# fan-ziqi/robot_lab

Measured on AMD Instinct MI355X. Metric: env-steps/sec (whole node) at 4096 envs/GPU, A1 Velocity-Rough, higher is better.
Workload: dtype f32; 1 GPU; RobotLab-Isaac-Velocity-Rough-Unitree-A1-v0, 4096 envs/GPU, random actions U(-1,1), seed 42+rank; envs_per_gpu=4096, parallelism=env-shard x1, step_kernel=specialised (spec_id 1), envs_per_wavefront=4

## Files before the change

__graft_entry__.py:

```python
from __future__ import annotations

import os
import subprocess
import sys

ROOT = os.path.dirname(os.path.abspath(__file__))
CSRC = os.path.join(ROOT, "robot_lab_amd", "csrc")
HIP_LIB = os.path.join(CSRC, "librl_env_hip.so")
EMU_DIR = os.path.join(ROOT, "tests", "emu")
EMU_LIB = os.path.join(EMU_DIR, "librl_env_emu.so")
HEADERS = ["rl_math.h", "env_tables.h", "env_step.h", "env_terms.h", "env_aos.h", "rl_env_host.h", "rl_env_capi.inl", "rl_env_kernels.h", "rl_env_sub.inl",
           "env_spec.h", "rl_env_spec.inl", "rl_env_specgen.h", os.path.join("spec", "env_specs_gen.h")]
ENV_SOURCES = ["rl_env.hip", "rl_env_sub1.hip", "rl_env_sub2.hip", "rl_env_sub8.hip"] + sorted(
    os.path.join("spec", f) for f in os.listdir(os.path.join(CSRC, "spec")) if f.startswith("rl_env_spec_") and f.endswith(".hip"))


def _stale(target, sources):
    if not os.path.isfile(target):
        return True
    t = os.path.getmtime(target)
    return any(os.path.getmtime(s) > t for s in sources)


_ONLY_MISSING = False
# ... 3 lines not shown
    return not os.path.isfile(target) if _ONLY_MISSING else _stale(target, sources)


VALIDATED_HIPCC = "HIP version: 7.2.26015-fc0010cf6a"
BUILD_INFO = os.path.join(CSRC, "build_info.json")


def _record_compiler(hipcc: str, extra: dict | None = None) -> None:
    import json

    try:
        ver = subprocess.run([hipcc, "--version"], capture_output=True, text=True, check=True).stdout.strip().splitlines()
    except (OSError, subprocess.CalledProcessError):
        ver = ["unknown"]
    ok = bool(ver) and ver[0].strip() == VALIDATED_HIPCC
    with open(BUILD_INFO, "w") as f:
        json.dump({"hipcc": hipcc, "version": ver[:2], "validated": VALIDATED_HIPCC, "matches_validated": ok,
                   "flags": " ".join(ENV_FLAGS), **(extra or {})}, f, indent=1)
    if not ok:
        print(f"[build] WARNING: hipcc reports {ver[0]!r}, the env library was validated with {VALIDATED_HIPCC!r}: run the GPU parity "
              f"tier and tests/test_gpu_canary.py before trusting this build", flush=True)


ENV_FLAGS = ["--offload-arch=gfx950", "-O3", "-fno-slp-vectorize", "-fno-signed-zeros", "-ffinite-math-only", "-mllvm", "-amdgpu-remove-redundant-endcf=false", "-std=c++17"]


def _abi_stamp_flag() -> str:
    if ROOT not in sys.path:
        sys.path.insert(0, ROOT)
    from robot_lab_amd import jit

    return jit.stamp_flag()


def _build_env_library(hipcc: str) -> None:
    import importlib.util
    import shutil
    import tempfile

    spec = importlib.util.spec_from_file_location("isa_exec_hazard", os.path.join(ROOT, "tools", "isa_exec_hazard.py"))
    chk = importlib.util.module_from_spec(spec)
    spec.loader.exec_module(chk)
    with tempfile.TemporaryDirectory(prefix="rl_env_build_") as tmp:
        procs = []
        for src in ENV_SOURCES:
            d = os.path.join(tmp, os.path.basename(src)[:-4])
            os.makedirs(d)
# ... 265 lines not shown
```

robot_lab_amd/csrc/env_step.h:

```cpp
#pragma once
#include <type_traits>

#include "env_spec.h"
#include "env_tables.h"

#if !defined(RL_NO_PK) && !defined(RL_PK)
#define RL_PK 1
#endif
#if defined(RL_PHASE_MARKS) && defined(__HIP_DEVICE_COMPILE__)
#define RL_PHASE(id, name) asm volatile("; PHASE " name)
#elif defined(RL_PHASE_CLOCK) && defined(__HIP_DEVICE_COMPILE__)
#define RL_PHASE(id, name) this->phase_stamp(id)
#define RL_PHASE_START() (this->ph_t0 = 0, this->ph_cur = 0)
#define RL_PHASE_CLOCK_ON 1
#else
#define RL_PHASE(id, name) ((void)0)
#endif
#ifndef RL_PHASE_START
#define RL_PHASE_START() ((void)0)
#endif
constexpr int RL_PHASE_ROW0 = 24;
constexpr int RL_PHASE_SLOTS = 32;

namespace rl {
// ... 83 lines not shown
struct TerrainPatch {
  float h00, h01, h10, h11, fx, fy;
};
struct TerrainBase {
  int cx, cy;
  float fx, fy;
  float lox, hix, loy, hiy;
};
RL_FN TerrainBase terrain_base(const Uni& u, float bx, float by) {
  TerrainBase b;
  if (u.is_plane) {
    b.cx = b.cy = 0;
    b.fx = b.fy = b.lox = b.hix = b.loy = b.hiy = 0.f;
    return b;
  }
  const double gx = ((double)bx - u.x0d) * u.inv_hd, gy = ((double)by - u.y0d) * u.inv_hd;
  const double cx = floor(gx), cy = floor(gy);
  b.cx = (int)cx; b.cy = (int)cy;
  b.fx = (float)(gx - cx); b.fy = (float)(gy - cy);
  b.lox = (float)(-b.cx); b.hix = (float)(u.nx - 2 - b.cx);
  b.loy = (float)(-b.cy); b.hiy = (float)(u.ny - 2 - b.cy);
  return b;
}
RL_FN TerrainPatch terrain_fetch(const Uni& u, const float* __restrict__ hf, const TerrainBase& tb, float dx, float dy) {
  TerrainPatch p;
  if (u.is_plane) {
    p.h00 = p.h01 = p.h10 = p.h11 = 0.f;
    p.fx = p.fy = 0.f;
    return p;
  }
  const float gx = tb.fx + dx * u.inv_hscale, gy = tb.fy + dy * u.inv_hscale;
  const float ox = clampf(floorf(gx), tb.lox, tb.hix), oy = clampf(floorf(gy), tb.loy, tb.hiy);
  p.fx = clampf(gx - ox, 0.f, 1.f);
  p.fy = clampf(gy - oy, 0.f, 1.f);
  const int ix = imin(imax(tb.cx + (int)ox, 0), u.nx - 2), iy = imin(imax(tb.cy + (int)oy, 0), u.ny - 2);
  if constexpr (TERRAIN_PAIRS) {
    const F4h r = ld4_a8(hf + (((uint32_t)ix * (uint32_t)u.ny + (uint32_t)iy) << 1));
    p.h00 = r.x; p.h10 = r.y; p.h01 = r.z; p.h11 = r.w;
  } else {
    const float* b = hf + (uint32_t)ix * (uint32_t)u.ny + (uint32_t)iy;
    F2 r0 = ld2(b), r1 = ld2(b + u.ny);
    p.h00 = r0.x; p.h01 = r0.y; p.h10 = r1.x; p.h11 = r1.y;
  }
  return p;
}
RL_FN TerrainPatch terrain_fetch(const Uni& u, const float* __restrict__ hf, float bx, float by, float dx, float dy) {
  return terrain_fetch(u, hf, terrain_base(u, bx, by), dx, dy);
}
RL_FN void terrain_eval(const Uni& u, const TerrainPatch& p, float& h, V3& n) {
  float hx0 = p.h00 + p.fx * (p.h10 - p.h00), hx1 = p.h01 + p.fx * (p.h11 - p.h01);
  h = hx0 + p.fy * (hx1 - hx0);
  float dzdx = ((1.f - p.fy) * (p.h10 - p.h00) + p.fy * (p.h11 - p.h01)) * u.inv_hscale;
  float dzdy = ((1.f - p.fx) * (p.h01 - p.h00) + p.fx * (p.h11 - p.h10)) * u.inv_hscale;
  float inv = frsqrt(dzdx * dzdx + dzdy * dzdy + 1.0f);
  n = {-dzdx * inv, -dzdy * inv, inv};
}
RL_FN float terrain_height(const TerrainPatch& p) {
  const float hx0 = p.h00 + p.fx * (p.h10 - p.h00), hx1 = p.h01 + p.fx * (p.h11 - p.h01);
// ... 2141 lines not shown
```

robot_lab_amd/csrc/env_terms.h:

```cpp
#pragma once
#include "env_spec.h"
#include "env_step.h"

namespace rl {

enum RewKind {
  REW_TRACK_LIN_VEL_XY_EXP = 0, REW_TRACK_ANG_VEL_Z_EXP, REW_LIN_VEL_Z_L2, REW_ANG_VEL_XY_L2, REW_JOINT_TORQUES_L2,
  REW_JOINT_ACC_L2, REW_JOINT_POS_LIMITS, REW_JOINT_POWER, REW_STAND_STILL, REW_JOINT_POS_PENALTY, REW_JOINT_MIRROR,
  REW_ACTION_RATE_L2, REW_UNDESIRED_CONTACTS, REW_CONTACT_FORCES, REW_FEET_CONTACT_WITHOUT_CMD, REW_FEET_HEIGHT_BODY,
  REW_UPWARD, REW_FEET_AIR_TIME, REW_FEET_AIR_TIME_VARIANCE, REW_FEET_SLIDE, REW_FEET_GAIT, REW_FLAT_ORIENTATION_L2,
  REW_IS_TERMINATED, REW_JOINT_DEVIATION_L1, REW_JOINT_VEL_L2, REW_FEET_CONTACT, REW_FEET_STUMBLE, REW_FEET_HEIGHT,
  REW_TRACK_LIN_VEL_XY_YAW_FRAME_EXP, REW_TRACK_ANG_VEL_Z_WORLD_EXP, REW_FEET_AIR_TIME_POSITIVE_BIPED,
  REW_HANDSTAND_FEET_HEIGHT_EXP, REW_HANDSTAND_FEET_ON_AIR, REW_HANDSTAND_FEET_AIR_TIME, REW_HANDSTAND_ORIENTATION_L2, REW_BASE_HEIGHT_L2, REW_WHEEL_VEL_PENALTY,
  REW_FEET_DISTANCE_Y_EXP, REW_FEET_DISTANCE_XY_EXP, REW_ACTION_MIRROR, REW_ACTION_SYNC
};
enum ObsKind {
  OBS_BASE_LIN_VEL = 0, OBS_BASE_ANG_VEL, OBS_PROJECTED_GRAVITY, OBS_VELOCITY_COMMANDS, OBS_JOINT_POS_REL,
  OBS_JOINT_VEL_REL, OBS_LAST_ACTION, OBS_HEIGHT_SCAN, OBS_JOINT_POS_REL_NO_WHEEL
};

enum { JS_TAU2 = 0, JS_ACC2, JS_QD2, JS_LIMIT, JS_POWER, JS_DEV1, JS_DEV2, JS_DA2, JS_Q, JS_ABSQD, JS_ROWS };
enum { BT_HMAX = 0, BT_CA, BT_CC, BT_LA, BT_LC, BT_FX, BT_FY, BT_FZ, BT_PX, BT_PY, BT_PZ, BT_VX, BT_VY, BT_VZ, BT_NF };
static_assert(JS_ROWS == REW_JS_ROWS && BT_NF == REW_BT_NF && BT_FX == REW_BT_NS, "reward tables: LDS sizing in env_tables.h");

// ... 276 lines not shown
        case REW_UNDESIRED_CONTACTS: f = a0 * gate; break;
        case REW_CONTACT_FORCES: f = a0; break;
        case REW_FEET_CONTACT_WITHOUT_CMD: f = a0 * (cmd_norm < 0.1f ? 1.f : 0.f) * gate; break;
        case REW_FEET_CONTACT: f = (a0 != R.p[0] ? 1.f : 0.f) * moving * gate; break;
        case REW_FEET_AIR_TIME: f = a0 * moving * gate; break;
        case REW_HANDSTAND_FEET_AIR_TIME: f = a0; break;
        case REW_FEET_STUMBLE: f = (a0 > 0.f ? 1.f : 0.f) * gate; break;
        case REW_FEET_HEIGHT_BODY: case REW_FEET_HEIGHT: f = a0 * moving * gate; break;
        case REW_FEET_SLIDE: f = a0 * gate; break;
        case REW_FEET_AIR_TIME_POSITIVE_BIPED: f = (a0 == 1.f ? fminf(mn, R.p[0]) : 0.f) * moving * gate; break;
        case REW_HANDSTAND_FEET_HEIGHT_EXP: f = fexp(-a0 * frcp(R.p[0])); break;
        case REW_HANDSTAND_FEET_ON_AIR: f = a0 == 0.f ? 1.f : 0.f; break;
        case REW_FEET_AIR_TIME_VARIANCE: {
          const float inv_n = frcp(a0), inv_den = frcp(fmaxf(a0 - 1.f, 1.f));
          f = ((a2 - a1 * a1 * inv_n) + (a4 - a3 * a3 * inv_n)) * inv_den * gate;
        } break;
        default: break;
      }
    } break;
  }
  return f;
}


template <class Ctx, class TP, class SP = NoSpec>
struct EnvProgram : EnvLane<Ctx, TP, SP> {
  using Base = EnvLane<Ctx, TP, SP>;
  using ChainTP = typename Base::ChainTP;
  static constexpr Layout LY = Base::LY;
  static constexpr int CL = TP::CL, NW = TP::NW, JX = TP::JX, NBS = TP::NBS;
  using Base::ctx; using Base::S; using Base::T; using Base::L; using Base::e; using Base::k; using Base::sub; using Base::li; using Base::Np;
  static constexpr int SUB = Base::SUB;
  static constexpr int LPE = Base::LPE;
  using Base::pos; using Base::quat; using Base::vlin; using Base::vang; using Base::q; using Base::qd; using Base::kp; using Base::kd;
  using Base::act; using Base::prev_act; using Base::tim; using Base::cf; using Base::hist_n; using Base::tau_app; using Base::qacc;
  using Base::extF; using Base::extT; using Base::base_com; using Base::wr_com;

  V3 cmd;
  float heading_target, cmd_time_left, metric_xy, metric_yaw, push_left;
  static constexpr bool DEFER_LOG = SUB > 1;
  static constexpr int NACC_M = (MAX_T + LPE - 1) / LPE;
  float log_sum[NACC_M], log_mxy, log_myaw;
  bool is_heading, is_standing;
  int level, ttype;
  V3 origin;
  long long ep_len;
// ... 682 lines not shown

  RL_FN void scanner_pose(float& cy, float& sy, V3& scan_p, bool chain_fresh) {
    if (NW == 0) {
      cy = yaw_c; sy = yaw_s; scan_p = {0.f, 0.f, pos.z};
      return;
    }
    M3 Rf;
    V3 pf;
    if (chain_fresh) {
      ChainTP C = this->new_chain();
      trunk_frame<TP>(C, T.scan_depth, Rf, pf);
    } else {
      RL_PHASE(31, "obs.kinematics");
      trunk_frame_of_pose<TP>(L, q, this->u.trunk_restart, T.scan_depth, Rf, pf);
      RL_PHASE(20, "observations");
    }
    const M3 Rs = mul(Rwb, Rf);
    const float hn = frsqrt(fmaxf(Rs.r0.x * Rs.r0.x + Rs.r1.x * Rs.r1.x, 1e-30f));
    cy = Rs.r0.x * hn; sy = Rs.r1.x * hn;
    const V3 so = mul(Rwb, pf + mul(Rf, V3{T.scan_pos[0], T.scan_pos[1], T.scan_pos[2]}));
    scan_p = {so.x, so.y, pos.z + so.z};
  }

  static constexpr int SCAN_RB = LPE >= 32 ? 6 : 12;
  struct ScanPatches {
    TerrainPatch tp[SCAN_RB];
    bool single_trip;
  };
  RL_FN int scan_ray_of_slot(int s, int scan_n, float cy, float sy) const {
    s = s < scan_n ? s : scan_n - 1;
#ifndef RL_SCAN_YAW_LANES
    return s;
#else
    const int snx = ctx.uniform_i(T.scan_nx);
    const float inv_sny = ctx.uniform(1.0f / (float)T.scan_ny);
    const int ixt = (int)(((float)s + 0.5f) * inv_sny), iyt = s - ixt * ctx.uniform_i(T.scan_ny);
    return fabsf(cy) > fabsf(sy) ? iyt * snx + ixt : s;
#endif
  }
  RL_FN void scan_fetch_trip(int r0, int scan_n, float cy, float sy, V3 scan_p, ScanPatches& sp) const {
    const TerrainBase tb = terrain_base(this->u, pos.x, pos.y);
    const int snx = ctx.uniform_i(T.scan_nx);
    const float inv_snx = ctx.uniform(1.0f / (float)T.scan_nx);
    const float res = T.scan_res, cx0 = 0.5f * (float)(T.scan_nx - 1), cy0 = 0.5f * (float)(T.scan_ny - 1);
#pragma unroll
    for (int i = 0; i < SCAN_RB; ++i) {
      const int r = scan_ray_of_slot(r0 + i * LPE, scan_n, cy, sy);
      int iy = (int)(((float)r + 0.5f) * inv_snx), ix = r - iy * snx;
      float lx = ((float)ix - cx0) * res, ly = ((float)iy - cy0) * res;
      sp.tp[i] = terrain_fetch(this->u, S.terrain, tb, scan_p.x + cy * lx - sy * ly, scan_p.y + sy * lx + cy * ly);
    }
  }
  RL_FN void scan_fetch(float cy, float sy, V3 scan_p, ScanPatches& sp) const {
    const int scan_n = ctx.uniform_i(T.scan_nx * T.scan_ny);
    const bool wanted = ctx.uniform_i(T.obs[0].scan_n + T.obs[1].scan_n) > 0;
    sp.single_trip = wanted && scan_n <= SCAN_RB * LPE;
#ifdef RL_ABL_NO_SCAN
    sp.single_trip = false;
#endif
    if (sp.single_trip) scan_fetch_trip(li, scan_n, cy, sy, scan_p, sp);
  }

  template <bool DIRECT, class GT>
  RL_FN void write_group(const GT& G, const float* F, float* stage, uint32_t noise_base, float cy, float sy, V3 scan_p, const ScanPatches& sp) {
    constexpr int NITC = (TP::OBS_NC + LPE - 1) / LPE;
#ifdef RL_ABL_NO_SCAN
    const int n_cols = ctx.uniform_i(G.n_cols), scan_off = ctx.uniform_i(G.scan_off), scan_n = 0;
#else
    const int n_cols = ctx.uniform_i(G.n_cols), scan_off = ctx.uniform_i(G.scan_off), scan_n = ctx.uniform_i(G.scan_n);
#endif
    const int dim = ctx.uniform_i(G.dim);
    const bool corrupt = !DIRECT && ctx.uniform_i(G.corrupt) != 0;
    {
      ObsColTab d[NITC];
      float f[NITC];
#pragma unroll
      for (int i = 0; i < NITC; ++i) {
        const int n = li + LPE * i;
        d[i] = G.col[n < n_cols ? n : 0];
      }
#pragma unroll
      for (int i = 0; i < NITC; ++i) f[i] = F[d[i].src];
#pragma unroll
      for (int i = 0; i < NITC; ++i) {
        const int n = li + LPE * i;
        if (n < n_cols) stage[n < scan_off ? n : n + scan_n] = corrupt ? f[i] : clampf(f[i], d[i].clip_lo, d[i].clip_hi) * d[i].scale;
      }
    }
    if (scan_n > 0) write_scan(stage, scan_off, scan_n, corrupt, ctx.uniform(G.scan.scale), ctx.uniform(G.scan.clip_lo), ctx.uniform(G.scan.clip_hi), cy, sy, scan_p, sp);
    if (corrupt) noise_pass(G, stage, noise_base, dim, scan_off, scan_n);
  }
  RL_FN void write_scan(float* stage, int scan_off, int scan_n, bool corrupt, float s_scale, float s_lo, float s_hi, float cy, float sy, V3 scan_p,
                        const ScanPatches& sp) {
    const float soff = T.scan_offset;
    if (sp.single_trip) {
#pragma unroll
      for (int i = 0; i < SCAN_RB; ++i) {
        const int sl = li + i * LPE, r = scan_ray_of_slot(sl, scan_n, cy, sy);
        const float v = scan_p.z - terrain_height(sp.tp[i]) - soff;
        if (sl < scan_n) stage[scan_off + r] = corrupt ? v : clampf(v, s_lo, s_hi) * s_scale;
      }
    } else {
      for (int r0 = li; r0 < scan_n; r0 += SCAN_RB * LPE) {
        ScanPatches one;
        scan_fetch_trip(r0, scan_n, cy, sy, scan_p, one);
#pragma unroll
        for (int i = 0; i < SCAN_RB; ++i) {
          const int sl = r0 + i * LPE, r = scan_ray_of_slot(sl, scan_n, cy, sy);
          const float v = scan_p.z - terrain_height(one.tp[i]) - soff;
          if (sl < scan_n) stage[scan_off + r] = corrupt ? v : clampf(v, s_lo, s_hi) * s_scale;
        }
      }
    }
  }
  template <class GT>
  RL_FN void noise_pass(const GT& G, float* stage, uint32_t noise_base, int dim, int scan_off, int scan_n) {
    ctx.group_sync();
    const int nblk = (dim + 3) >> 2;
#pragma unroll 1
    for (int b = li; b < nblk; b += LPE) {
      float un[4];
      uniform01x4(S.seed, (uint32_t)e, S.step_counter, STREAM_NOISE, (noise_base >> 2) + (uint32_t)b, un);
// ... 146 lines not shown
      int b = L.slot_body[s];
      if (b >= 0 && (s != 0 || L.owns_base_body) && this->owns_slot(s)) {
        float* o = S.dbg_cforce + ((size_t)e * T.n_bodies + b) * 3;
        const F4 fs = cf.ld(s);
        o[0] = live * fs.x; o[1] = live * fs.y; o[2] = live * fs.z;
      }
    }
  }
  RL_FN bool out_of_bounds() const {
    if (!T.term_oob || T.is_plane) return false;
    const float mw = (float)T.num_rows * T.tile_size + 2.f * T.border, mh = (float)T.num_cols * T.tile_size + 2.f * T.border;
    return fabsf(pos.x) > 0.5f * mw - T.oob_buffer || fabsf(pos.y) > 0.5f * mh - T.oob_buffer;
  }

  RL_FN void step() { step_front<false>(); }
  RL_FN void step_head() { step_front<true>(); }
  RL_FN void step_tail() {
    this->load();
    load_task();
    derive();
    const bool terminated = S.terminated[e] != 0, time_out = S.time_out[e] != 0;
    const bool t_oob = out_of_bounds();
    const bool t_timeout = T.term_time_out && ep_len >= (long long)T.max_episode_length;
    step_back<true>(terminated, time_out, t_timeout, t_oob, terminated);
  }

  template <bool HEAD>
  RL_FN void step_front() {
    constexpr size_t LOG_SLOT_WORDS = (size_t)LOG_PARTS * LOG_SIZE;
    const int log_tl = ctx.tile(), log_wl = ctx.env_in_tile() * LPE + li;
    float* log_pv = S.log + (size_t)((S.step_counter - 1u) & (uint32_t)(LOG_RING - 1)) * LOG_SLOT_WORDS;
    const float* log_pp = S.log + (size_t)((S.step_counter - 2u) & (uint32_t)(LOG_RING - 1)) * LOG_SLOT_WORDS;
    float log_fresh = 0.f, log_word = 0.f;
    if (log_tl < LOG_PARTS) {
      for (int p = 0; p < LOG_PARTS; ++p) log_fresh += log_pv[p * LOG_SIZE + LOG_FRESH];
      log_word = log_pp[log_tl * LOG_SIZE + log_wl];
    }
    float a_in[JX];
    {
      const float* arow = S.action_in + (size_t)(e < S.N ? e : 0) * T.D;
#pragma unroll
      for (int j = 0; j < JX; ++j) {
        const int jid = L.joint_id[j];
        a_in[j] = arow[TP::PAD && jid < 0 ? 0 : jid];
      }
    }
    RL_PHASE_START();
// ... 16 lines not shown
#pragma unroll
    for (int j = 0; j < JX; ++j) {
      prev_act[j] = act[j];
      const float a = (e < S.N && (!TP::PAD || L.joint_id[j] >= 0)) ? a_in[j] : 0.f;
      act[j] = a;
      float pr = clampf(a * L.a_scale[j] + L.a_off[j], L.a_lo[j], L.a_hi[j]);
      q_tgt[j] = L.action_is_vel[j] ? 0.f : pr;
      qd_tgt[j] = L.action_is_vel[j] ? pr : 0.f;
    }
#ifdef RL_ABL_SUBSTEPS
    if constexpr (Base::ABA) {
      this->substeps_aba(q_tgt, qd_tgt, RL_ABL_SUBSTEPS);
    } else
#endif
    if constexpr (Base::ABA) {
      this->substeps_aba(q_tgt, qd_tgt, T.decimation);
    } else {
      this->self_load();
      for (int s = 0; s < T.decimation; ++s) this->substep_aba_trunk(q_tgt, qd_tgt);
    }
    RL_PHASE(15, "terminations");
    ep_len += 1;
    derive();
    if constexpr (NW > 0) {
      ChainTP Cf = this->new_chain();
      this->kinematics(Cf);
      ctx.group_sync();
    }

    bool t_timeout = T.term_time_out && ep_len >= (long long)T.max_episode_length;
    const bool t_oob = out_of_bounds();
    bool t_illegal = false;
    if (T.term_illegal) {
      const uint64_t ill_mask = T.illegal_body_mask;
      const float ill_thr = T.illegal_threshold;
      float c = 0.f;
#pragma unroll
      for (int i = 0; i < Base::MAXOWN; ++i) {
        const int so = this->own[i], s = so < 0 ? 0 : so;
        const float h = hist_max(s);
        const bool bit = body_bit(ill_mask, s);
        c += (so >= 0 && bit && h > ill_thr) ? 1.f : 0.f;
      }
      t_illegal = ctx.esum(c) > 0.f;
    }
    bool terminated = t_illegal, time_out = t_timeout || t_oob;
// ... 8 lines not shown
    else rew = compute_rewards(terminated, fold_done);
#endif
    RL_PHASE(19, "resets+commands+push");
    if (li == 0) {
      S.reward[e] = rew;
      S.terminated[e] = terminated ? 1 : 0;
      S.time_out[e] = time_out ? 1 : 0;
      if (S.ro_rewards != nullptr && e < S.N) {
        if (S.ro_values != nullptr) {
          S.ro_rewards[e] = time_out ? fmaf(S.ro_gamma, S.ro_values[e], rew) : rew;
          S.ro_dones[e] = (terminated || time_out) ? 1 : 0;
        } else {
          S.ro_rewards[e] = rew;
          S.ro_dones[e] = ((terminated || time_out) ? 1 : 0) | (time_out ? 2 : 0);
        }
      }
    }
    if constexpr (HEAD) {
      collect_cmd_levels(terminated || time_out);
      write_dbg_views((terminated || time_out) ? 0.f : 1.f);
      this->store();
      store_task();
    } else {
      step_back<false>(terminated, time_out, t_timeout, t_oob, t_illegal, fold_done);
    }
  }

  template <bool TAIL>
  RL_FN void step_back(const bool terminated, const bool time_out, const bool t_timeout, const bool t_oob, const bool t_illegal, const bool sums_folded = false) {
    if (terminated || time_out) {
      if (!(DEFER_LOG && sums_folded) && li == 0 && e < S.N) {
        if (t_timeout) ctx.atomic_add(log_slot() + LOG_TERM_TIMEOUT, 1.f);
        if (t_oob) ctx.atomic_add(log_slot() + LOG_TERM_OOB, 1.f);
        if (t_illegal) ctx.atomic_add(log_slot() + LOG_TERM_ILLEGAL, 1.f);
      }
      reset_env(true, sums_folded);
      derive();
      RL_PHASE(19, "resets+commands+push");
    }
    if constexpr (!TAIL) write_dbg_views((terminated || time_out) ? 0.f : 1.f);
#ifdef RL_SCAN_EARLY
    ScanAhead scanA;
    scan_ahead(!TAIL && !ctx.any(terminated || time_out), scanA);
#endif
    RL_PHASE(29, "commands");
    {
      const float inv_max_step = T.step_dt * frcp(T.cmd_resample[1]);
      float ex = cmd.x - lin_b.x, ey = cmd.y - lin_b.y;
      metric_xy += fsqrt(ex * ex + ey * ey) * inv_max_step;
      metric_yaw += fabsf(cmd.z - ang_b.z) * inv_max_step;
      cmd_time_left -= T.step_dt;
      if (cmd_time_left <= 0.f) {
        cmd_time_left = U(STREAM_COMMAND, 6, T.cmd_resample[0], T.cmd_resample[1]);
        resample_command(STREAM_COMMAND, 0);
      }
      if (T.cmd_heading && is_heading) {
        const float heading_w = atan2f(yaw_s, yaw_c);
        cmd.z = clampf(T.cmd_heading_stiffness * wrap_to_pi(heading_target - heading_w), T.cur_ang ? S.cmd_levels[CL_ANG_Z] : T.cmd_range[2][0],
                       T.cur_ang ? S.cmd_levels[CL_ANG_Z + 1] : T.cmd_range[2][1]);
      }
      if (is_standing) cmd = {0.f, 0.f, 0.f};
    }
    RL_PHASE(30, "push");
    if (T.ev_push) {
      push_left -= T.step_dt;
      if (push_left < 1e-6f) {
        push_left = U(STREAM_PUSH, 6, T.push_interval[0], T.push_interval[1]);
        vlin += V3{U(STREAM_PUSH, 0, T.push_vel[0][0], T.push_vel[0][1]), U(STREAM_PUSH, 1, T.push_vel[1][0], T.push_vel[1][1]),
                   U(STREAM_PUSH, 2, T.push_vel[2][0], T.push_vel[2][1])};
        vang += V3{U(STREAM_PUSH, 3, T.push_vel[3][0], T.push_vel[3][1]), U(STREAM_PUSH, 4, T.push_vel[4][0], T.push_vel[4][1]),
                   U(STREAM_PUSH, 5, T.push_vel[5][0], T.push_vel[5][1])};
      }
    }
    RL_PHASE(23, "store");
#ifndef RL_ABL_NO_STORE
    this->store();
    store_task();
#endif
    RL_PHASE(20, "observations");
#ifndef RL_ABL_NO_OBS
#ifdef RL_SCAN_EARLY
    observations(scanA);
#else
    observations(!TAIL && !ctx.any(terminated || time_out));
#endif
#endif
#ifndef RL_ABL_NO_LOG
    if constexpr (DEFER_LOG) {
      if (sums_folded && e < S.N) {
        float* slot = log_slot();
        int n_rew;
        if constexpr (SP::ON) n_rew = SP::N_REW;
        else n_rew = T.n_rewards;
#pragma unroll
        for (int i = 0; i < NACC_M; ++i) {
          const int t = li + LPE * i;
          if (t < n_rew) ctx.atomic_add(slot + LOG_EP_SUM0 + t, log_sum[i]);
        }
        if (li == 0) {
          ctx.atomic_add(slot + LOG_RESET_COUNT, 1.0f);
          ctx.atomic_add(slot + LOG_FRESH, 1.0f);
          ctx.atomic_add(slot + LOG_METRIC_XY, log_mxy);
          ctx.atomic_add(slot + LOG_METRIC_YAW, log_myaw);
          if (t_timeout) ctx.atomic_add(slot + LOG_TERM_TIMEOUT, 1.f);
          if (t_oob) ctx.atomic_add(slot + LOG_TERM_OOB, 1.f);
          if (t_illegal) ctx.atomic_add(slot + LOG_TERM_ILLEGAL, 1.f);
        }
      }
// ... 23 lines not shown
```

robot_lab_amd/csrc/rl_env.hip:

```cpp
#include <dlfcn.h>

#include <mutex>

#include "rl_env_kernels.h"
#include "rl_env_host.h"
#include "rl_env_specgen.h"

#define RL_ENV_PLUGINS 1
#ifndef RL_ENV_ABI_STAMP
#define RL_ENV_ABI_STAMP "unstamped"
#endif
namespace {
struct SpecPlugin {
  int id = 0;
  int (*matches)(const void* tables) = nullptr;
  int (*launch)(const void* cfg, const void* S, const void* T, int sub, size_t lds1, void* stream) = nullptr;
};
std::vector<SpecPlugin>& spec_plugins() {
  static std::vector<SpecPlugin> v;
  return v;
}
std::mutex& spec_plugins_mutex() {
  static std::mutex m;
  return m;
// ... 125 lines not shown
        case 4: need[0] = lds_need<TopoQuad4, 4>(T); need[1] = lds_need<TopoQuad4, 2>(T); need[2] = lds_need<TopoQuad4, 1>(T); break;
        case 104: need[0] = lds_need<TopoQuad4M, 4>(T); need[1] = lds_need<TopoQuad4M, 2>(T); need[2] = lds_need<TopoQuad4M, 1>(T); break;
        default: break;
      }
      const int subs[3] = {4, 2, 1};
      const double cost[3] = {1.0, 1.45, 2.29};
      double best = 0.0, t[3] = {0.0, 0.0, 0.0};
      for (int i = 0; i < 3; ++i) {
        if (need[i] == 0 || need[i] > 160 * 1024) continue;
        const size_t per_cu = (tb + 4 * (need[i] - tb) <= 160 * 1024) ? 4 : std::min<size_t>(4, (160 * 1024) / need[i]);
        const double slots = (double)n_cu * (double)per_cu, waves = (double)(Npad / (16 / subs[i]));
        t[i] = cost[i] * std::ceil(waves / slots);
        if (best == 0.0 || t[i] < 0.97 * best) { best = t[i]; sub = subs[i]; }
      }
      if (std::getenv("RL_ENV_DEBUG"))
        fprintf(stderr, "rl_env: %d envs: rounds x cost of 4 / 2 / 1 lanes per limb = %.2f / %.2f / %.2f (LDS per wavefront %zu / %zu / %zu B, tables %zu B) -> %d lane(s) per limb\n",
                Npad, t[0], t[1], t[2], need[0], need[1], need[2], tb, sub);
    }
    return 16 / sub;
  }
  size_t lds_bytes = 0;
  template <class TP, int SUB>
  static size_t lds_need(const Tables& T) {
    const LdsPlan P = lds_plan<TP, SUB>(T.policy_dim, T.critic_dim, direct_group(T, 0), direct_group(T, 1), T.D, T.n_bodies, T.rew_ext_mask, T.n_rewards);
    return staged_bytes(T) + (size_t)P.words * 4;
  }
  int configure(const Tables& T) {
    const int key = (T.CL + (T.merged ? 100 : 0) + (T.NW > 3 ? 200 : 0) + (T.rotpad ? 400 : 0)) * 10 + sub;
    switch (key) {
      case 31: lds_bytes = lds_need<TopoQuad3, 1>(T); break;
      case 32: lds_bytes = lds_need<TopoQuad3, 2>(T); break;
      case 34: lds_bytes = lds_need<TopoQuad3, 4>(T); break;
      case 41: lds_bytes = lds_need<TopoQuad4, 1>(T); break;
      case 42: lds_bytes = lds_need<TopoQuad4, 2>(T); break;
      case 44: lds_bytes = lds_need<TopoQuad4, 4>(T); break;
      case 1041: lds_bytes = lds_need<TopoQuad4M, 1>(T); break;
      case 1042: lds_bytes = lds_need<TopoQuad4M, 2>(T); break;
      case 1044: lds_bytes = lds_need<TopoQuad4M, 4>(T); break;
      case 4041: lds_bytes = lds_need<TopoQuad4R, 1>(T); break;
      case 4042: lds_bytes = lds_need<TopoQuad4R, 2>(T); break;
      case 4044: lds_bytes = lds_need<TopoQuad4R, 4>(T); break;
      case 71:
        err = "the one-lane-per-limb mapping (RL_ENV_SUB=1) of the trunk + limbs instance needs more LDS than a CU has";
        return -1;
      case 74: lds_bytes = lds_need<TopoG1, 4>(T); break;
      case 78: lds_bytes = lds_need<TopoG1, 8>(T); break;
      case 2078: lds_bytes = lds_need<TopoGR, 8>(T); break;
// ... 98 lines not shown
```

robot_lab_amd/csrc/rl_env_kernels.h:

```cpp
#pragma once
#include <hip/hip_runtime.h>

#include <algorithm>
#include <cmath>
#include <cstdlib>
#include <mutex>
#include <string>

#define RL_FN __host__ __device__ __forceinline__
#include "env_aos.h"
#include "env_terms.h"

namespace {

using namespace rl;

template <int CTRL>
__device__ inline float dpp(float v) {
  return __int_as_float(__builtin_amdgcn_update_dpp(0, __float_as_int(v), CTRL, 0xF, 0xF, false));
}
template <int CTRL>
__device__ inline float dpp_move(float v) {
  return __int_as_float(__builtin_amdgcn_update_dpp(0, __float_as_int(v), CTRL, 0xF, 0xF, true));
}
// ... 133 lines not shown
      auto b = [](float v) { return dpp_move<J | (J << 2) | (J << 4) | (J << 6)>(v); };
      return M3{{b(m.r0.x), b(m.r0.y), b(m.r0.z)}, {b(m.r1.x), b(m.r1.y), b(m.r1.z)}, {b(m.r2.x), b(m.r2.y), b(m.r2.z)}};
    } else return leg_bcast_m3<J>(m);
  }
  template <int J>
  __device__ __forceinline__ M3 leg_bcast_m3(const M3& m) const {
    return M3{{leg_bcast<J>(m.r0.x), leg_bcast<J>(m.r0.y), leg_bcast<J>(m.r0.z)},
              {leg_bcast<J>(m.r1.x), leg_bcast<J>(m.r1.y), leg_bcast<J>(m.r1.z)},
              {leg_bcast<J>(m.r2.x), leg_bcast<J>(m.r2.y), leg_bcast<J>(m.r2.z)}};
  }
  template <int D, int N>
  __device__ __forceinline__ void sub_shr(float (&w)[N]) const {
    static_assert(SUB == 8 && D >= 1 && D < 8, "eight sub-lanes per limb");
#pragma unroll
    for (int i = 0; i < N; ++i) w[i] = dpp_move<0x110 + D>(w[i]);
  }
  __device__ float gshfl(float v, int leg) const { return __shfl(v, (lane & ~(LPE - 1)) | (leg * SUB) | (lane & (SUB - 1))); }
  __device__ void atomic_add(float* p, float v) const { atomicAdd(p, v); }
  __device__ float* obs_stage(int g) const { return stage[g] + env_in_tile() * dim[g]; }
  __device__ float* rew_stage() const { return rstage + env_in_tile() * rsdim; }
  __device__ float* feat_stage() const { return fstage + env_in_tile() * fdim; }
  __device__ float* rew_tab() const { return stage[0] + env_in_tile() * rtdim; }
  __device__ float* rand_tab() const { return stage[0] + env_in_tile() * RESET_RAND_WORDS; }
  __device__ static void wave_sync() {
#ifdef RL_SYNCTHREADS
    __syncthreads();
#else
    __builtin_amdgcn_fence(__ATOMIC_ACQ_REL, "wavefront");
    __builtin_amdgcn_wave_barrier();
#endif
  }
  __device__ void group_sync() const { wave_sync(); }
  __device__ void flush_obs(float* out, int d, int g) const {
    wave_sync();
    const int n4 = (EPT * d) >> 2;
    if (((EPT * d) & 3) == 0) {
      const float4* src = reinterpret_cast<const float4*>(stage[g]);
      float4* dst = reinterpret_cast<float4*>(out + (size_t)wtile * EPT * d);
      for (int i = lane; i < n4; i += 64) dst[i] = src[i];
    } else {
      float* dst = out + (size_t)wtile * EPT * d;
      for (int i = lane; i < EPT * d; i += 64) dst[i] = stage[g][i];
    }
    wave_sync();
  }
};

struct LdsPlan {
  int s0w, s1w;
  int fdim, rtdim, rsdim;
  int lb0, lbrec0, envs, tail;
  int rstage, stage0, stage1, fstage;
  int words;
};
template <class TP, int SUB>
RL_FN LdsPlan lds_plan(int policy_dim, int critic_dim, bool direct0, bool direct1, int D, int n_bodies, uint64_t rew_ext_mask, int n_rewards) {
  constexpr int EPT = 64 / (NLANE * SUB), LIMBS = 64 / SUB;
  using LS = typename LsFor<TP, SUB>::type;
  constexpr int STASH_WORDS = LsFor<TP, SUB>::STASH * LsFor<TP, SUB>::type::SSW * 64;
  constexpr int LB_FREE = TP::NW > 0 ? LbLayout<TP>::RECW * LIMBS : 0;
  LdsPlan P;
  P.s0w = (SUB == 1 && direct0) ? 0 : (EPT * policy_dim + 3) & ~3;
  P.s1w = (SUB == 1 && direct1) ? 0 : (EPT * critic_dim + 3) & ~3;
  P.fdim = feat_count(D);
  P.rtdim = rew_tab_words(D, n_bodies, rew_ext_mask);
  P.rsdim = rew_stage_words(n_rewards);
  int region = P.s0w + P.s1w + EPT * P.fdim;
  if (region < EPT * P.rtdim) P.s1w += EPT * P.rtdim - region, region = EPT * P.rtdim;
  if (SUB > 1 && region < EPT * RESET_RAND_WORDS) P.s1w += EPT * RESET_RAND_WORDS - region, region = EPT * RESET_RAND_WORDS;
  P.lb0 = LS::WORDS * 64;
  P.lbrec0 = P.lb0 + LbLayout<TP>::CHAINW * LIMBS;
  P.envs = P.lb0 + LbLayout<TP>::WORDS * LIMBS;
  P.tail = P.envs + EPT * LbLayout<TP>::ENV_WORDS;
  const bool alias = TP::NW == 0 && STASH_WORDS > 0 && EPT * P.rsdim + region <= STASH_WORDS;
  const bool alias_lb = TP::NW > 0 && EPT * P.rsdim + region <= LB_FREE;
  P.rstage = alias ? LS::CT * 64 : (alias_lb ? P.lbrec0 : P.tail);
  P.stage0 = P.rstage + EPT * P.rsdim;
  P.stage1 = P.stage0 + P.s0w;
  P.fstage = P.stage1 + P.s1w;
  P.words = (alias || alias_lb) ? P.tail : P.tail + EPT * P.rsdim + region;
  P.words = (P.words + 3) & ~3;
  return P;
}

extern __shared__ float4 smem4[];

#ifndef RL_LB
#define RL_LB(w) 256
#endif
template <class TP, int RESET, int SUB, int WGW, class SP = NoSpec>
__global__ __launch_bounds__(RL_LB(WGW)) void env_kernel(KState S, const void* __restrict__ Tgv, uint32_t wave_words) {
  using Ctx = WaveCtx<SUB>;
  using Tables = TablesT<TP>;
  const Tables* __restrict__ Tg = static_cast<const Tables*>(Tgv);
  float* smem = reinterpret_cast<float*>(smem4);
  Tables* Tl = reinterpret_cast<Tables*>(smem);
  const int lane = threadIdx.x & 63, wv = threadIdx.x >> 6;
  S.step_counter += *S.step_base;
  {
    const float4* src = reinterpret_cast<const float4*>(Tg);
    float4* dst = reinterpret_cast<float4*>(Tl);
    constexpr int TPB = 64 * WGW;
    constexpr int NIT = ((int)(sizeof(Tables) / 16) + TPB - 1) / TPB;
    const int n4 = (int)(S.table_bytes >> 4);
    float4 tmp[NIT];
#pragma unroll
    for (int it = 0; it < NIT; ++it) {
      const int i = (int)threadIdx.x + TPB * it;
      tmp[it] = src[i < n4 ? i : n4 - 1];
    }
#pragma unroll
    for (int it = 0; it < NIT; ++it) {
      const int i = (int)threadIdx.x + TPB * it;
      if (i < n4) dst[i] = tmp[it];
    }
  }
  if (WGW > 1) __syncthreads();
  else Ctx::wave_sync();
  const int TAB_F = (int)(S.table_bytes >> 2);
  const LdsPlan P = lds_plan<TP, SUB>(Tl->policy_dim, Tl->critic_dim, direct_group(*Tl, 0), direct_group(*Tl, 1), Tl->D, Tl->n_bodies, Tl->rew_ext_mask, Tl->n_rewards);
  Ctx ctx;
  ctx.T = Tl;
  ctx.Tg = Tgv;
  ctx.dim[0] = Tl->policy_dim;
  ctx.dim[1] = Tl->critic_dim;
  ctx.lscratch = smem + TAB_F + (WGW > 1 ? wv * wave_words : 0u);
  ctx.wtile = (int)blockIdx.x * WGW + wv;
  if (WGW > 1 && ctx.wtile >= S.Npad / Ctx::EPT) return;
  ctx.lbchain = ctx.lscratch + P.lb0 + (lane / SUB) * LbLayout<TP>::CHAINW;
  ctx.lbrec = ctx.lscratch + P.lbrec0 + (lane / SUB) * LbLayout<TP>::RECW;
  ctx.lbrec_stride = LbLayout<TP>::RECW;
  ctx.envs = ctx.lscratch + P.envs + (lane / Ctx::LPE) * LbLayout<TP>::ENV_WORDS;
  ctx.fdim = P.fdim;
  ctx.rtdim = P.rtdim;
  ctx.rsdim = P.rsdim;
  ctx.rstage = ctx.lscratch + P.rstage;
  ctx.stage[0] = ctx.lscratch + P.stage0;
  ctx.stage[1] = ctx.lscratch + P.stage1;
  ctx.fstage = ctx.lscratch + P.fstage;
  ctx.lane = lane;
  EnvProgram<Ctx, TP, SP> prog(ctx, S);
  if (RESET == 1)
    prog.reset_entry();
  else if (RESET == 2)
    prog.step_head();
  else
    prog.step();
}


struct LaunchCfg {
  int device = 0, n_cu = 256;
  int wg_waves = 4;
  bool wg_force = false;
};

template <class TP, int SUB, int WGW, class SP = NoSpec>
hipError_t launch_w(const LaunchCfg& cfg, const KState& S, const void* T, size_t lds1, hipStream_t st) {
  const int tiles = S.Npad / (16 / SUB);
  dim3 grid((tiles + WGW - 1) / WGW), block(64 * WGW);
  const uint32_t wave_words = (uint32_t)((lds1 - S.table_bytes) >> 2);
  const size_t lds = S.table_bytes + (size_t)WGW * (lds1 - S.table_bytes);
// ... 66 lines not shown
```

robot_lab_amd/jit.py:

```python
from __future__ import annotations

import ctypes as C
import hashlib
import os
import subprocess
import sys

_HERE = os.path.dirname(os.path.abspath(__file__))
CSRC = os.path.join(_HERE, "csrc")
ROOT = os.path.dirname(_HERE)
ENV_FLAGS = ["--offload-arch=gfx950", "-O3", "-fno-slp-vectorize", "-fno-signed-zeros", "-ffinite-math-only", "-mllvm", "-amdgpu-remove-redundant-endcf=false", "-std=c++17"]
_registered: dict[str, int] = {}


def abi_stamp() -> str:
    h = hashlib.sha256()
    names = sorted(f for f in os.listdir(CSRC) if f.endswith((".h", ".inl"))) + [os.path.join("spec", "env_specs_gen.h")]
    for n in names:
        with open(os.path.join(CSRC, n), "rb") as f:
            h.update(n.encode() + b"\0" + f.read())
    with open(os.path.join(ROOT, "include", "rl_env.h"), "rb") as f:
        h.update(f.read())
    return h.hexdigest()[:16]


def stamp_flag(stamp: str | None = None) -> str:
    return '-DRL_ENV_ABI_STAMP="%s"' % (stamp or abi_stamp())


def enabled(flag) -> bool:
    return bool(flag) if flag is not None else os.environ.get("RL_ENV_JIT", "1") == "1"


def cache_dir() -> str:
# ... 99 lines not shown
```

Before: 131.8 million env-steps/s.

## Gather height-scan terrain samples into LDS via async global_load_lds issued early

Adds an LDS gather path for the height-scan observation. Per-ray terrain cell indices are computed, and the four corner heights are issued as global_load_lds_dword direct-to-LDS loads right after derive(), before kinematics and rewards. They are waited on only when the observations are built, so terrain fetch latency overlaps other step work. It reserves extra LDS per workgroup, which may reduce occupancy, and uses inline asm with m0 and waitcnt handling that could interact badly with other outstanding loads.

```diff
diff --git a/__graft_entry__.py b/__graft_entry__.py
--- a/__graft_entry__.py
+++ b/__graft_entry__.py
@@ -49,7 +49,7 @@
               f"tier and tests/test_gpu_canary.py before trusting this build", flush=True)
 
 
-ENV_FLAGS = ["--offload-arch=gfx950", "-O3", "-fno-slp-vectorize", "-fno-signed-zeros", "-ffinite-math-only", "-mllvm", "-amdgpu-remove-redundant-endcf=false", "-std=c++17"]
+ENV_FLAGS = ["--offload-arch=gfx950", "-O3", "-fno-slp-vectorize", "-fno-signed-zeros", "-ffinite-math-only", "-mllvm", "-amdgpu-remove-redundant-endcf=false", "-Wno-inline-asm", "-std=c++17"]
 
 
 def _abi_stamp_flag() -> str:
diff --git a/robot_lab_amd/csrc/env_step.h b/robot_lab_amd/csrc/env_step.h
--- a/robot_lab_amd/csrc/env_step.h
+++ b/robot_lab_amd/csrc/env_step.h
@@ -129,6 +129,28 @@
   b.loy = (float)(-b.cy); b.hiy = (float)(u.ny - 2 - b.cy);
   return b;
 }
+struct TerrainCell {
+  int ix, iy;
+  float fx, fy;
+};
+RL_FN TerrainCell terrain_cell(const Uni& u, const TerrainBase& tb, float dx, float dy) {
+  TerrainCell c;
+  const float gx = tb.fx + dx * u.inv_hscale, gy = tb.fy + dy * u.inv_hscale;
+  const float ox = clampf(floorf(gx), tb.lox, tb.hix), oy = clampf(floorf(gy), tb.loy, tb.hiy);
+  c.fx = clampf(gx - ox, 0.f, 1.f);
+  c.fy = clampf(gy - oy, 0.f, 1.f);
+  c.ix = imin(imax(tb.cx + (int)ox, 0), u.nx - 2);
+  c.iy = imin(imax(tb.cy + (int)oy, 0), u.ny - 2);
+  return c;
+}
+RL_FN void terrain_cell_words(const Uni& u, const TerrainCell& c, uint32_t (&w)[4]) {
+  const uint32_t b = (uint32_t)c.ix * (uint32_t)u.ny + (uint32_t)c.iy;
+  if constexpr (TERRAIN_PAIRS) {
+    w[0] = b << 1; w[2] = w[0] + 1u; w[1] = w[0] + 2u; w[3] = w[0] + 3u;
+  } else {
+    w[0] = b; w[1] = b + 1u; w[2] = b + (uint32_t)u.ny; w[3] = w[2] + 1u;
+  }
+}
 RL_FN TerrainPatch terrain_fetch(const Uni& u, const float* __restrict__ hf, const TerrainBase& tb, float dx, float dy) {
   TerrainPatch p;
   if (u.is_plane) {
@@ -136,11 +158,10 @@
     p.fx = p.fy = 0.f;
     return p;
   }
-  const float gx = tb.fx + dx * u.inv_hscale, gy = tb.fy + dy * u.inv_hscale;
-  const float ox = clampf(floorf(gx), tb.lox, tb.hix), oy = clampf(floorf(gy), tb.loy, tb.hiy);
-  p.fx = clampf(gx - ox, 0.f, 1.f);
-  p.fy = clampf(gy - oy, 0.f, 1.f);
-  const int ix = imin(imax(tb.cx + (int)ox, 0), u.nx - 2), iy = imin(imax(tb.cy + (int)oy, 0), u.ny - 2);
+  const TerrainCell c = terrain_cell(u, tb, dx, dy);
+  p.fx = c.fx;
+  p.fy = c.fy;
+  const int ix = c.ix, iy = c.iy;
   if constexpr (TERRAIN_PAIRS) {
     const F4h r = ld4_a8(hf + (((uint32_t)ix * (uint32_t)u.ny + (uint32_t)iy) << 1));
     p.h00 = r.x; p.h10 = r.y; p.h01 = r.z; p.h11 = r.w;
diff --git a/robot_lab_amd/csrc/env_terms.h b/robot_lab_amd/csrc/env_terms.h
--- a/robot_lab_amd/csrc/env_terms.h
+++ b/robot_lab_amd/csrc/env_terms.h
@@ -322,6 +322,25 @@
   return f;
 }
 
+
+constexpr int scan_rays_per_lane(int lpe) { return lpe >= 32 ? 6 : 12; }
+template <class C, class = void>
+struct ctx_has_lds_gather : std::false_type {};
+template <class C>
+struct ctx_has_lds_gather<C, std::void_t<decltype(C::LDS_GATHER)>> : std::integral_constant<bool, C::LDS_GATHER> {};
+template <class SP>
+constexpr bool spec_carries_scan() {
+  if constexpr (SP::ON) {
+    for (int g = 0; g < 2; ++g)
+      for (int i = 0; i < SP::N_OBS[g]; ++i)
+        if (SP::OBS[g][i].kind == OBS_HEIGHT_SCAN) return true;
+    return false;
+  } else return true;
+}
+template <class TT>
+RL_FN int scan_gather_rays(const TT& T) {
+  return (T.obs[0].scan_n + T.obs[1].scan_n > 0 && !T.is_plane) ? T.scan_nx * T.scan_ny : 0;
+}
 
 template <class Ctx, class TP, class SP = NoSpec>
 struct EnvProgram : EnvLane<Ctx, TP, SP> {
@@ -1050,7 +1069,8 @@
     scan_p = {so.x, so.y, pos.z + so.z};
   }
 
-  static constexpr int SCAN_RB = LPE >= 32 ? 6 : 12;
+  static constexpr int SCAN_RB = scan_rays_per_lane(LPE);
+  static constexpr bool SCAN_LDS = ctx_has_lds_gather<Ctx>::value && NW == 0 && LPE == 16 && spec_carries_scan<SP>();
   struct ScanPatches {
     TerrainPatch tp[SCAN_RB];
     bool single_trip;
@@ -1079,6 +1099,27 @@
       sp.tp[i] = terrain_fetch(this->u, S.terrain, tb, scan_p.x + cy * lx - sy * ly, scan_p.y + sy * lx + cy * ly);
     }
   }
+  RL_FN void scan_gather_trip(int scan_n, float cy, float sy, V3 scan_p, ScanPatches& sp) const {
+    if constexpr (SCAN_LDS) {
+      const TerrainBase tb = terrain_base(this->u, pos.x, pos.y);
+      const int snx = ctx.uniform_i(T.scan_nx);
+      const float inv_snx = ctx.uniform(1.0f / (float)T.scan_nx);
+      const float res = T.scan_res, cx0 = 0.5f * (float)(T.scan_nx - 1), cy0 = 0.5f * (float)(T.scan_ny - 1);
+#pragma unroll
+      for (int i = 0; i < SCAN_RB; ++i) {
+        const int r = scan_ray_of_slot(li + i * LPE, scan_n, cy, sy);
+        int iy = (int)(((float)r + 0.5f) * inv_snx), ix = r - iy * snx;
+        float lx = ((float)ix - cx0) * res, ly = ((float)iy - cy0) * res;
+        const TerrainCell c = terrain_cell(this->u, tb, scan_p.x + cy * lx - sy * ly, scan_p.y + sy * lx + cy * ly);
+        uint32_t w[4];
+        terrain_cell_words(this->u, c, w);
+        sp.tp[i].fx = c.fx;
+        sp.tp[i].fy = c.fy;
+#pragma unroll
+        for (int h = 0; h < 4; ++h) ctx.gather_issue(4 * i + h, S.terrain, w[h]);
+      }
+    }
+  }
   RL_FN void scan_fetch(float cy, float sy, V3 scan_p, ScanPatches& sp) const {
     const int scan_n = ctx.uniform_i(T.scan_nx * T.scan_ny);
     const bool wanted = ctx.uniform_i(T.obs[0].scan_n + T.obs[1].scan_n) > 0;
@@ -1086,7 +1127,13 @@
 #ifdef RL_ABL_NO_SCAN
     sp.single_trip = false;
 #endif
-    if (sp.single_trip) scan_fetch_trip(li, scan_n, cy, sy, scan_p, sp);
+    if constexpr (SCAN_LDS) {
+      sp.single_trip = sp.single_trip && ctx.has_gather();
+      ctx.gather_open();
+      if (sp.single_trip) scan_gather_trip(scan_n, cy, sy, scan_p, sp);
+    } else {
+      if (sp.single_trip) scan_fetch_trip(li, scan_n, cy, sy, scan_p, sp);
+    }
   }
 
   template <bool DIRECT, class GT>
@@ -1122,10 +1169,16 @@
                         const ScanPatches& sp) {
     const float soff = T.scan_offset;
     if (sp.single_trip) {
+      if constexpr (SCAN_LDS) ctx.gather_wait();
 #pragma unroll
       for (int i = 0; i < SCAN_RB; ++i) {
         const int sl = li + i * LPE, r = scan_ray_of_slot(sl, scan_n, cy, sy);
-        const float v = scan_p.z - terrain_height(sp.tp[i]) - soff;
+        TerrainPatch p = sp.tp[i];
+        if constexpr (SCAN_LDS) {
+          p.h00 = ctx.gather_word(4 * i + 0); p.h01 = ctx.gather_word(4 * i + 1);
+          p.h10 = ctx.gather_word(4 * i + 2); p.h11 = ctx.gather_word(4 * i + 3);
+        }
+        const float v = scan_p.z - terrain_height(p) - soff;
         if (sl < scan_n) stage[scan_off + r] = corrupt ? v : clampf(v, s_lo, s_hi) * s_scale;
       }
     } else {
@@ -1318,7 +1371,8 @@
     const bool terminated = S.terminated[e] != 0, time_out = S.time_out[e] != 0;
     const bool t_oob = out_of_bounds();
     const bool t_timeout = T.term_time_out && ep_len >= (long long)T.max_episode_length;
-    step_back<true>(terminated, time_out, t_timeout, t_oob, terminated);
+    ScanAhead scanA;
+    step_back<true>(terminated, time_out, t_timeout, t_oob, terminated, false, scanA, false);
   }
 
   template <bool HEAD>
@@ -1381,6 +1435,9 @@
     RL_PHASE(15, "terminations");
     ep_len += 1;
     derive();
+    ScanAhead scanA;
+    constexpr bool SCAN_EARLY = SCAN_LDS && !HEAD;
+    if constexpr (SCAN_EARLY) scan_ahead(true, scanA);
     if constexpr (NW > 0) {
       ChainTP Cf = this->new_chain();
       this->kinematics(Cf);
@@ -1435,12 +1492,13 @@
       this->store();
       store_task();
     } else {
-      step_back<false>(terminated, time_out, t_timeout, t_oob, t_illegal, fold_done);
+      step_back<false>(terminated, time_out, t_timeout, t_oob, t_illegal, fold_done, scanA, SCAN_EARLY);
     }
   }
 
   template <bool TAIL>
-  RL_FN void step_back(const bool terminated, const bool time_out, const bool t_timeout, const bool t_oob, const bool t_illegal, const bool sums_folded = false) {
+  RL_FN void step_back(const bool terminated, const bool time_out, const bool t_timeout, const bool t_oob, const bool t_illegal, const bool sums_folded, ScanAhead& scanA,
+                       const bool scan_issued) {
     if (terminated || time_out) {
       if (!(DEFER_LOG && sums_folded) && li == 0 && e < S.N) {
         if (t_timeout) ctx.atomic_add(log_slot() + LOG_TERM_TIMEOUT, 1.f);
@@ -1452,10 +1510,13 @@
       RL_PHASE(19, "resets+commands+push");
     }
     if constexpr (!TAIL) write_dbg_views((terminated || time_out) ? 0.f : 1.f);
-#ifdef RL_SCAN_EARLY
-    ScanAhead scanA;
-    scan_ahead(!TAIL && !ctx.any(terminated || time_out), scanA);
-#endif
+    const bool chain_fresh = !TAIL && !ctx.any(terminated || time_out);
+    if constexpr (SCAN_LDS) {
+      if (!scan_issued || !chain_fresh) {
+        if (scan_issued) ctx.gather_wait();
+        scan_ahead(chain_fresh, scanA);
+      }
+    }
     RL_PHASE(29, "commands");
     {
       const float inv_max_step = T.step_dt * frcp(T.cmd_resample[1]);
@@ -1492,11 +1553,10 @@
 #endif
     RL_PHASE(20, "observations");
 #ifndef RL_ABL_NO_OBS
-#ifdef RL_SCAN_EARLY
-    observations(scanA);
+    if constexpr (SCAN_LDS) observations(scanA);
+    else observations(chain_fresh);
 #else
-    observations(!TAIL && !ctx.any(terminated || time_out));
-#endif
+    if constexpr (SCAN_LDS) ctx.gather_wait();
 #endif
 #ifndef RL_ABL_NO_LOG
     if constexpr (DEFER_LOG) {
diff --git a/robot_lab_amd/csrc/rl_env.hip b/robot_lab_amd/csrc/rl_env.hip
--- a/robot_lab_amd/csrc/rl_env.hip
+++ b/robot_lab_amd/csrc/rl_env.hip
@@ -171,7 +171,7 @@
   size_t lds_bytes = 0;
   template <class TP, int SUB>
   static size_t lds_need(const Tables& T) {
-    const LdsPlan P = lds_plan<TP, SUB>(T.policy_dim, T.critic_dim, direct_group(T, 0), direct_group(T, 1), T.D, T.n_bodies, T.rew_ext_mask, T.n_rewards);
+    const LdsPlan P = lds_plan<TP, SUB>(T.policy_dim, T.critic_dim, direct_group(T, 0), direct_group(T, 1), T.D, T.n_bodies, T.rew_ext_mask, T.n_rewards, scan_gather_rays(T), (uint32_t)staged_bytes(T));
     return staged_bytes(T) + (size_t)P.words * 4;
   }
   int configure(const Tables& T) {
diff --git a/robot_lab_amd/csrc/rl_env_kernels.h b/robot_lab_amd/csrc/rl_env_kernels.h
--- a/robot_lab_amd/csrc/rl_env_kernels.h
+++ b/robot_lab_amd/csrc/rl_env_kernels.h
@@ -179,6 +179,20 @@
   __device__ float* feat_stage() const { return fstage + env_in_tile() * fdim; }
   __device__ float* rew_tab() const { return stage[0] + env_in_tile() * rtdim; }
   __device__ float* rand_tab() const { return stage[0] + env_in_tile() * RESET_RAND_WORDS; }
+#ifdef RL_SCAN_LDS_OFF
+  static constexpr bool LDS_GATHER = false;
+#else
+  static constexpr bool LDS_GATHER = true;
+#endif
+  float* gather;
+  uint32_t gather_at;
+  __device__ bool has_gather() const { return gather != nullptr; }
+  __device__ void gather_issue(int row, const float* ubase, uint32_t word) const {
+    asm volatile("s_mov_b32 m0, %2\n\ts_nop 0\n\tglobal_load_lds_dword %0, %1" : : "v"(word << 2), "s"(ubase), "s"(gather_at + (uint32_t)row * 256u) : "memory", "m0");
+  }
+  __device__ static void gather_open() { __builtin_amdgcn_s_waitcnt(0x0F70); }
+  __device__ static void gather_wait() { asm volatile("s_waitcnt vmcnt(0)" ::: "memory"); }
+  __device__ float gather_word(int row) const { return gather[row * 64 + lane]; }
   __device__ static void wave_sync() {
 #ifdef RL_SYNCTHREADS
     __syncthreads();
@@ -208,10 +222,11 @@
   int fdim, rtdim, rsdim;
   int lb0, lbrec0, envs, tail;
   int rstage, stage0, stage1, fstage;
+  int gather;
   int words;
 };
 template <class TP, int SUB>
-RL_FN LdsPlan lds_plan(int policy_dim, int critic_dim, bool direct0, bool direct1, int D, int n_bodies, uint64_t rew_ext_mask, int n_rewards) {
+RL_FN LdsPlan lds_plan(int policy_dim, int critic_dim, bool direct0, bool direct1, int D, int n_bodies, uint64_t rew_ext_mask, int n_rewards, int scan_rays, uint32_t table_bytes) {
   constexpr int EPT = 64 / (NLANE * SUB), LIMBS = 64 / SUB;
   using LS = typename LsFor<TP, SUB>::type;
   constexpr int STASH_WORDS = LsFor<TP, SUB>::STASH * LsFor<TP, SUB>::type::SSW * 64;
@@ -237,6 +252,14 @@
   P.fstage = P.stage1 + P.s1w;
   P.words = (alias || alias_lb) ? P.tail : P.tail + EPT * P.rsdim + region;
   P.words = (P.words + 3) & ~3;
+  P.gather = -1;
+  if constexpr (WaveCtx<SUB>::LDS_GATHER && TP::NW == 0 && NLANE * SUB == 16) {
+    constexpr int GW = 4 * scan_rays_per_lane(NLANE * SUB) * 64;
+    if (scan_rays > 0 && scan_rays <= scan_rays_per_lane(NLANE * SUB) * NLANE * SUB && (size_t)table_bytes + 4 * (size_t)(P.words + GW) * 4 <= (size_t)160 * 1024) {
+      P.gather = P.words;
+      P.words += GW;
+    }
+  }
   return P;
 }
 
@@ -275,7 +298,7 @@
   if (WGW > 1) __syncthreads();
   else Ctx::wave_sync();
   const int TAB_F = (int)(S.table_bytes >> 2);
-  const LdsPlan P = lds_plan<TP, SUB>(Tl->policy_dim, Tl->critic_dim, direct_group(*Tl, 0), direct_group(*Tl, 1), Tl->D, Tl->n_bodies, Tl->rew_ext_mask, Tl->n_rewards);
+  const LdsPlan P = lds_plan<TP, SUB>(Tl->policy_dim, Tl->critic_dim, direct_group(*Tl, 0), direct_group(*Tl, 1), Tl->D, Tl->n_bodies, Tl->rew_ext_mask, Tl->n_rewards, scan_gather_rays(*Tl), S.table_bytes);
   Ctx ctx;
   ctx.T = Tl;
   ctx.Tg = Tgv;
@@ -295,6 +318,8 @@
   ctx.stage[0] = ctx.lscratch + P.stage0;
   ctx.stage[1] = ctx.lscratch + P.stage1;
   ctx.fstage = ctx.lscratch + P.fstage;
+  ctx.gather = __builtin_amdgcn_readfirstlane(P.gather) >= 0 ? ctx.lscratch + P.gather : nullptr;
+  ctx.gather_at = (uint32_t)__builtin_amdgcn_readfirstlane((int)(uint32_t)reinterpret_cast<uintptr_t>(ctx.gather));
   ctx.lane = lane;
   EnvProgram<Ctx, TP, SP> prog(ctx, S);
   if (RESET == 1)
diff --git a/robot_lab_amd/jit.py b/robot_lab_amd/jit.py
--- a/robot_lab_amd/jit.py
+++ b/robot_lab_amd/jit.py
@@ -9,7 +9,7 @@
 _HERE = os.path.dirname(os.path.abspath(__file__))
 CSRC = os.path.join(_HERE, "csrc")
 ROOT = os.path.dirname(_HERE)
-ENV_FLAGS = ["--offload-arch=gfx950", "-O3", "-fno-slp-vectorize", "-fno-signed-zeros", "-ffinite-math-only", "-mllvm", "-amdgpu-remove-redundant-endcf=false", "-std=c++17"]
+ENV_FLAGS = ["--offload-arch=gfx950", "-O3", "-fno-slp-vectorize", "-fno-signed-zeros", "-ffinite-math-only", "-mllvm", "-amdgpu-remove-redundant-endcf=false", "-Wno-inline-asm", "-std=c++17"]
 _registered: dict[str, int] = {}
 
 
```

Result: slower. 116.8 million env-steps/s (-11.4%).
